# metno/gridpp

Hardware: AMD Instinct MI355X
Metric: grid cells/sec for optimal_interpolation, 4000x4000 grid, 10k obs (higher is better)
Workload: dtype f32 (rho, distances) + f64 (local solve)

## Files before the change

### gridpp_amd/csrc/oi_union.h

```cpp
#pragma once
#include "oi_common.h"

#pragma clang fp contract(off)

struct OiArgs {
    const float *gx, *gy, *gz, *gelev, *glaf, *bg, *bvar;
    float *out, *out_var;
    int C, ny, nx, tiles_x, ntiles, tiled2d;
    int wshift;
    ScanArgs s;
    const float4* ogeo;
    const float4* oaux;
    const float4* saux;
    int S, allow_extrap;
    int* err;
    unsigned long long* counters;
    const int* in_list;
    const int* in_count;
    int* out_list;
    int* out_count;
    int nrun;
    int tile0, tile_n;
    int* tail_count;
    const unsigned char* skip_flags;
    int level;
    const int* parent_count;
    int debug;
    int no_bulk_cert;
    int pair_solo;
    int* big_list;
    int* big_count;
    unsigned long long* big_keys;
    double* big_mat;
    int* huge_list;
    int* huge_count;
    unsigned long long* huge_keys;
    double* huge_mat;
    int huge_kcap, huge_ncap;
    unsigned* pair_sel;
    int* pair_n;
};

#define GPP_NSLOT 512
#define BIG_CAND 8192
#define BIG_N 512
#define BIG_NL 104
#define ERR_OVERFLOW 1
#define ERR_SINGULAR 2

__device__ __forceinline__ int nth_set_bit(unsigned long long mask, int m) {
    int pos = 0;
#pragma unroll
    for(int w = 32; w > 0; w >>= 1) {
        unsigned long long lowmask = (w == 32) ? 0xffffffffull : ((1ull << w) - 1ull);
        int c = __popcll((mask >> pos) & lowmask);
        if(m >= c) { m -= c; pos += w; }
    }
    return pos;
}

#ifdef GPP_UNION_STATS
#define UNION_STATS true
#else
#define UNION_STATS false
#endif
#ifdef GPP_UNION_PROFILE
#define UPROF(i) do { const unsigned long long t_ = __builtin_amdgcn_s_memtime(); if(lane == 0) L.prof[i] += (unsigned)(t_ - tprev); tprev = t_; } while(0)
#else
#define UPROF(i) do { } while(0)
#endif

template <int NC> struct UnionCfg;
template <> struct UnionCfg<32> {
    static constexpr int WCAP = 40;
    static constexpr int MAXU = 40;
    static constexpr int SOLVE = 1024;
#ifndef GPP_UNION_PERSIST
#define GPP_UNION_PERSIST 0
#endif
#ifndef GPP_UNION_WPB
#define GPP_UNION_WPB 2
#endif
    static constexpr int WPB = GPP_UNION_WPB;
    template <bool PLAIN> static constexpr bool persistent() { return PLAIN && GPP_UNION_PERSIST != 0; }
};
template <> struct UnionCfg<48> {
    static constexpr int WCAP = 56;
    static constexpr int MAXU = 56;
    static constexpr int SOLVE = 1792;
    static constexpr int WPB = 2;
    template <bool PLAIN> static constexpr bool persistent() { return false; }
};
template <> struct UnionCfg<64> {
    static constexpr int WCAP = 64;
    static constexpr int MAXU = 62;
    static constexpr int SOLVE = 2240;
    static constexpr int WPB = 2;
    template <bool PLAIN> static constexpr bool persistent() { return false; }
};
constexpr int U_MAXE = 12;
constexpr int U_MAXM = 6;

__device__ __forceinline__ unsigned union_xcd_order(const unsigned b, const unsigned nblocks) {
    const unsigned g = b & ~15u;
    if(g + 16u > nblocks) return b;
    const unsigned r = b & 15u;
    return g + ((r & 7u) << 1) + (r >> 3);
}

template <int NC>
struct UnionLds {
    static constexpr int U_WCAP = UnionCfg<NC>::WCAP, U_MAXU = UnionCfg<NC>::MAXU, U_SOLVE = UnionCfg<NC>::SOLVE;
    union {
        float rho[U_WCAP][64];
        struct {
            double solve[U_SOLVE];
            float erho[U_MAXE][64];
        } f;
    };
    int wpos[U_WCAP];
    int worig[U_WCAP];
#ifdef GPP_UNION_PROFILE
    unsigned prof[24];
#endif
    union {
        struct {
            float4 orec[U_MAXU];
            float olaf[U_MAXU];
        };
        double late[8][9];
    };
};

struct PairLds {
    int pos[2][UnionCfg<32>::WCAP];
    unsigned long long core[2];
    int state[2];
    int ok[2];
    float dmax, dmin;
};

#ifndef GPP_UNION_COLS
#define GPP_UNION_COLS 0
#endif
template <int NC, bool COLS>
__device__ __forceinline__ int union_solve_doubles(const int c, const int nE) {
    if constexpr(COLS) return c * (c + nE + 1) - c * (c - 1) / 2 + c + nE * nE + nE;
    else return c * (c + 1) / 2 + 2 * c + nE * (c | 1) + nE * nE + nE + 3;
}
__device__ __forceinline__ double rsqrt_nr(const double a) {
    double rs = __builtin_amdgcn_rsq(a);
    rs = rs * (1.5 - 0.5 * a * rs * rs);
    rs = rs * (1.5 - 0.5 * a * rs * rs);
    return rs;
}

template <bool PLAIN, bool LIST, int NC, bool PAIR = false, bool SP = false>
__device__ __forceinline__ void union_item(const OiArgs& a, int tile, int sub, const int shift, UnionLds<NC>& L, const int lane,
                                           const bool partner = false, const int pw = 0, const int lead = 0, UnionLds<NC>* const Lall = nullptr, PairLds* const PP = nullptr) {
    constexpr int U_WCAP = UnionCfg<NC>::WCAP, U_MAXU = UnionCfg<NC>::MAXU, U_SOLVE = UnionCfg<NC>::SOLVE;
    static_assert(!PAIR || (NC == 32 && !LIST), "the pair form exists for the first pass of the 32-column kernel only");
    static_assert(!SP || (PLAIN && NC == 32 && !PAIR), "the spatially varying form exists for the 32-column Barnes kernel only");
    tile = __builtin_amdgcn_readfirstlane(tile); sub = __builtin_amdgcn_readfirstlane(sub);
#ifdef GPP_UNION_PROFILE
    if(lane < 24) L.prof[lane] = 0u;
    unsigned long long tprev = __builtin_amdgcn_s_memtime();
#endif
    int cell = -1;
    if(a.tiled2d) {
        int ty = tile / a.tiles_x, tx = tile - ty * a.tiles_x;
        int y = ty * (64 >> a.wshift) + (lane >> a.wshift), x = (tx << a.wshift) + (lane & ((1 << a.wshift) - 1));
        if(y < a.ny && x < a.nx) cell = y * a.nx + x;
    }
    else {
        int c = tile * 64 + lane;
        if(c < a.C) cell = c;
    }
    if(LIST && (lane >> shift) != sub) cell = -1;
    float gx = 0, gy = 0, gz = 0, ge = NAN, gl = NAN, bg = NAN, bvar = 1.0f;
    if(cell >= 0) {
        gx = a.gx[cell]; gy = a.gy[cell]; gz = a.gz[cell]; ge = a.gelev[cell]; gl = a.glaf[cell];
        bg = a.bg[cell];
        if(a.bvar) bvar = a.bvar[cell];
    }
    const bool active = cell >= 0 && d_valid(bg);
    DevStructure st = a.s.st;
    const ScanArgs& sa = a.s;
    float sa_inv_s = sa.inv_s;
    if constexpr(SP) { if(cell >= 0) d_structure_at(st, st.cell_idx ? st.cell_idx[cell] : cell); }
    else if constexpr(!LIST) asm volatile("" : "+s"(st.h), "+s"(st.v), "+s"(st.w), "+s"(st.R), "+s"(sa_inv_s));

    UPROF(0);
    const float R = st.R;
    const int K = sa.K;
    const float h2 = st.h * st.h;
    const bool prune = PLAIN || st.kh == SK_BARNES;
    const float pa = sa.axis_a == 0 ? gx : (sa.axis_a == 1 ? gy : gz);
    const float pb = sa.axis_b == 1 ? gy : (sa.axis_b == 2 ? gz : gx);
    const float amin_t = wave_min(active ? pa : INFINITY), amax_t = wave_max(active ? pa : -INFINITY);
    const float bmin_t = wave_min(active ? pb : INFINITY), bmax_t = wave_max(active ? pb : -INFINITY);
    float emin_t = -INFINITY, emax_t = INFINITY, lmin_t = -INFINITY, lmax_t = INFINITY, kv2 = 0.0f, kw2 = 0.0f;
    if constexpr(PLAIN && !SP) {
        if(d_valid(st.v) && st.v != 0.0f && d_valid(st.h) && st.h != 0.0f) {
            emin_t = wave_min(active ? (d_valid(ge) ? ge : -INFINITY) : INFINITY); emax_t = wave_max(active ? (d_valid(ge) ? ge : INFINITY) : -INFINITY);
            kv2 = (st.h / st.v) * (st.h / st.v) * 0.9999f;
        }
        if(d_valid(st.w) && st.w != 0.0f && d_valid(st.h) && st.h != 0.0f) {
            lmin_t = wave_min(active ? (d_valid(gl) ? gl : -INFINITY) : INFINITY); lmax_t = wave_max(active ? (d_valid(gl) ? gl : INFINITY) : -INFINITY);
            kw2 = (st.h / st.w) * (st.h / st.w) * 0.9999f;
        }
    }
    int cnt = 0;
    unsigned long long mine = 0ull;
    unsigned long long alloc = 0ull;
    bool fb = false;
    bool cert = false;
    constexpr unsigned long long FULL = U_WCAP >= 64 ? ~0ull : ((1ull << (U_WCAP & 63)) - 1ull);
#pragma unroll
    for(int w = 0; w < U_WCAP; ++w) L.rho[w][lane] = INFINITY;
    auto live_mask = [&]() { return wave_or64(mine); };
    auto bulk_own = [&](const bool ok, const int s) {
        const unsigned okm = ok ? ~0u : 0u;
        const unsigned long long bit = 1ull << s;
        mine = ((unsigned long long)d_and_or_sc(okm, (unsigned)(bit >> 32), (unsigned)(mine >> 32)) << 32) | d_and_or_sc(okm, (unsigned)bit, (unsigned)mine);
        cnt -= (int)okm;
    };
    auto worst_slot = [&](float& r0, int& s0, bool& multi) {
        constexpr int NG = U_WCAP / 8;
        float gm[NG];
#pragma unroll
        for(int g = 0; g < NG; ++g) {
            float v[8];
#pragma unroll
            for(int j = 0; j < 8; ++j) v[j] = L.rho[8 * g + j][lane];
            gm[g] = fminf(fminf(fminf(v[0], v[1]), fminf(v[2], v[3])), fminf(fminf(v[4], v[5]), fminf(v[6], v[7])));
        }
        r0 = gm[0];
#pragma unroll
        for(int g = 1; g < NG; ++g) r0 = fminf(r0, gm[g]);
        int gs = 0, ng = 0;
#pragma unroll
        for(int g = 0; g < NG; ++g) { const bool eq = gm[g] == r0; gs = eq ? g : gs; ng += eq ? 1 : 0; }
        const float* const grp = &L.rho[0][lane] + gs * (8 * 64);
        float v[8];
#pragma unroll
        for(int j = 0; j < 8; ++j) v[j] = grp[j * 64];
        int sj = 0, nin = 0;
#pragma unroll
        for(int j = 0; j < 8; ++j) { const bool eq = v[j] == r0; sj = eq ? j : sj; nin += eq ? 1 : 0; }
        s0 = 8 * gs + sj;
        multi = ng > 1 || nin > 1;
    };
    if(wave_ballot(active) != 0ull) {
        const float sbin = 1.0f / sa_inv_s;
        int tby0 = (int)floorf((bmin_t - sa.bmin) * sa_inv_s), tby1 = (int)floorf((bmax_t - sa.bmin) * sa_inv_s);
        tby0 = __builtin_amdgcn_readfirstlane(min(max(tby0, 0), sa.nby - 1));
        tby1 = __builtin_amdgcn_readfirstlane(min(max(tby1, tby0), sa.nby - 1));
        int tbx0 = (int)floorf((amin_t - sa.amin) * sa_inv_s), tbx1 = (int)floorf((amax_t - sa.amin) * sa_inv_s);
        tbx0 = __builtin_amdgcn_readfirstlane(min(max(tbx0, 0), sa.nbx - 1));
        tbx1 = __builtin_amdgcn_readfirstlane(min(max(tbx1, tbx0), sa.nbx - 1));
        const float lox = gx - R, hix = gx + R, loy = gy - R, hiy = gy + R, loz = gz - R, hiz = gz + R;
        const float near_r = R - 4.76837158e-7f * (fabsf(gx) + fabsf(gy) + fabsf(gz) + R);
        float wr = 0.0f;
        int ws = 0;
        unsigned wo = 0u;
        const float thr2_R = R * R * 1.000001f + 1e-30f;
        float thr2 = active ? thr2_R : -1.0f;
        float bud2 = active ? INFINITY : -1.0f;

        const float ca = 0.5f * (amin_t + amax_t), cb = 0.5f * (bmin_t + bmax_t);
        const float rad = 0.5f * d_sqrt_raw((amax_t - amin_t) * (amax_t - amin_t) + (bmax_t - bmin_t) * (bmax_t - bmin_t)) * 1.001f + 1e-30f;
        auto proj_d2 = [&](const float4& rec) {
            const float ra = sa.axis_a == 0 ? rec.x : (sa.axis_a == 1 ? rec.y : rec.z);
            const float rb = sa.axis_b == 1 ? rec.y : (sa.axis_b == 2 ? rec.z : rec.x);
            return (ra - ca) * (ra - ca) + (rb - cb) * (rb - cb);
        };
        auto wave_lim2 = [&]() {
            const float t2 = __int_as_float(__builtin_amdgcn_readfirstlane(__float_as_int(wave_max(thr2))));
            if(t2 < 0.0f) return -1.0f;
            const float lim = (d_sqrt_raw(t2) + rad) * 1.0001f;
            return lim * lim;
        };

        const bool eprune = PLAIN && (kv2 != 0.0f || kw2 != 0.0f);
        auto wave_bud2 = [&]() { return eprune ? __int_as_float(__builtin_amdgcn_readfirstlane(__float_as_int(wave_max(bud2)))) : INFINITY; };
        auto keep = [&](const float pd, const float4& rec, const float2& met, const float lim2, const float B2) {
            bool k = pd <= lim2;
            if(eprune && B2 < INFINITY) {
                const float sd = fmaxf(d_sqrt_raw(pd) * 0.9999f - rad, 0.0f);
                const float dz = fmaxf(fmaxf(emin_t - rec.w, rec.w - emax_t), 0.0f), dl = fmaxf(fmaxf(lmin_t - met.x, met.x - lmax_t), 0.0f);
                k = k && (sd * sd + kv2 * dz * dz + kw2 * dl * dl <= B2);
            }
            return k;
        };

        const bool hv = d_valid(st.v) && st.v != 0.0f, hw = d_valid(st.w) && st.w != 0.0f, hh = d_valid(st.h) && st.h != 0.0f;
// ... 401 lines not shown
                if(UNION_STATS && lane == 0) atomicAdd(&a.counters[12], (unsigned long long)min(64, total - base));
                run_chunk(rec, met, pos, wave_ballot(keep(pd, rec, met, lim2, B2)));
            }
            const int nidx = 32 * (b + 1);
            if(nidx >= n0) {
                const int rn = 1 + ((nidx - n0) >> 1);
                const float t2n = __int_as_float(__builtin_amdgcn_readfirstlane(__float_as_int(wave_max(thr2))));
                const float gapn = (rn > 1) ? (float)(rn - 1) * sbin * 0.999f : 0.0f;
                if(t2n < 0.0f || gapn * gapn > t2n) break;
                if(tby0 - rn < 0 && tby1 + rn >= sa.nby) break;
            }
        }
    }

    UPROF(4);
    const unsigned long long upd = wave_ballot(cnt > 0);
    unsigned long long coreM = 0ull, extM = 0ull;
    int c = 0, nE = 0, u = 0;
    int m = 0;
    unsigned elist = 0u;
    if(!fb && upd != 0ull) {
        const bool up = cnt > 0;
        const unsigned long long unionM = wave_or64(up ? mine : 0ull);
        coreM = wave_and64(up ? mine : ~0ull);
        extM = unionM & ~coreM;
        if constexpr(UNION_STATS) {
            unsigned long long held = 0ull;
            for(int w = 0; w < U_WCAP; ++w) held |= (L.rho[w][lane] < INFINITY ? 1ull : 0ull) << w;
            if(wave_ballot(held != mine) != 0ull && lane == 0) atomicAdd(&a.counters[13], 1ull);
        }
    }
    int myslot = 0, mypos = 0;
    bool paired = false;
    if constexpr(PAIR) {
        if(partner) {
            PairLds& P = *PP;
            __builtin_amdgcn_fence(__ATOMIC_RELEASE, "wavefront");
            __builtin_amdgcn_wave_barrier();
            __builtin_amdgcn_fence(__ATOMIC_ACQUIRE, "wavefront");
            if(lane < U_WCAP) P.pos[pw][lane] = (((coreM | extM) >> lane) & 1ull) ? L.wpos[lane] : -1;
            if(lane == 0) { P.core[pw] = coreM; P.state[pw] = fb ? 2 : (upd == 0ull ? 1 : 0); }
            UPROF(11);
            __syncthreads();
            UPROF(12);
            if(P.state[0] == 0 && P.state[1] == 0) {
                const int pa = lane < U_WCAP ? P.pos[0][lane] : -1, pb = lane < U_WCAP ? P.pos[1][lane] : -1;
                int partB = -1, partA = -1;
#pragma unroll
                for(int t = 0; t < U_WCAP; ++t) {
                    const int qa = P.pos[0][t], qb = P.pos[1][t];
                    partB = (qb == pa) ? t : partB;
                    partA = (qa == pb) ? t : partA;
                }
                partB = pa >= 0 ? partB : -1;
                partA = pb >= 0 ? partA : -1;
                const unsigned long long coreA = P.core[0], coreB = P.core[1];
                const unsigned long long liveA = wave_ballot(pa >= 0);
                const unsigned long long pcore = wave_ballot(pa >= 0 && ((coreA >> lane) & 1ull) != 0ull && partB >= 0 && ((coreB >> (partB & 63)) & 1ull) != 0ull);
                const unsigned long long pextA = liveA & ~pcore;
                const unsigned long long bonly = wave_ballot(pb >= 0 && partA < 0);
                const int c2 = __popcll(pcore), nEa = __popcll(pextA), nE2 = nEa + __popcll(bonly), u2 = c2 + nE2;
                const bool fits = u2 <= U_MAXU && nE2 <= U_MAXE && union_solve_doubles<NC, (NC == 32 && GPP_UNION_COLS != 0) || SP>(c2, nE2) <= U_SOLVE;
                int sA = -1, sB = -1;
                {
                    const unsigned long long mk = lane < c2 ? pcore : (lane < c2 + nEa ? pextA : bonly);
                    const int idx = lane < c2 ? lane : (lane < c2 + nEa ? lane - c2 : lane - c2 - nEa);
                    const int sl = nth_set_bit(mk, idx);
                    if(lane < c2 + nEa) sA = sl; else if(lane < u2) sB = sl;
                }
                const int pbs = __shfl(partB, sA < 0 ? 0 : sA);
                if(sA >= 0) sB = pbs;
                const int posA = P.pos[0][sA < 0 ? 0 : sA], posB = P.pos[1][sB < 0 ? 0 : sB];
                const int slot2 = pw == 0 ? sA : sB, pos2 = sA >= 0 ? posA : posB;
                int m2 = 0;
                unsigned el2 = 0u;
                if(fits) {
#pragma unroll
                    for(int ai = 0; ai < U_MAXE; ++ai) {
                        if(ai < nE2) {
                            const int sl = __builtin_amdgcn_readlane(slot2, c2 + ai);
                            const bool sel = sl >= 0 && L.rho[sl < 0 ? 0 : sl][lane] < INFINITY;
                            if(sel) { el2 |= (unsigned)ai << (4 * (m2 & 7)); m2++; }
                        }
                    }
                }
                const bool ok = fits && wave_ballot(m2 > U_MAXM) == 0ull;
                if(lane == 0) P.ok[pw] = ok ? 1 : 0;
                UPROF(13);
                __syncthreads();
                UPROF(14);
                paired = P.ok[0] != 0 && P.ok[1] != 0;
                if(paired) { c = c2; nE = nE2; u = u2; m = m2; elist = el2; myslot = slot2; mypos = pos2; }
            }
        }
    }
    if(!paired && !fb && upd != 0ull) {
        c = __popcll(coreM); nE = __popcll(extM); u = c + nE;
        if(u > U_MAXU || nE > U_MAXE || union_solve_doubles<NC, (NC == 32 && GPP_UNION_COLS != 0) || SP>(c, nE) > U_SOLVE) {
            fb = true;
            if(UNION_STATS && lane == 0) atomicAdd(&a.counters[u > U_MAXU ? 5 : (nE > U_MAXE ? 6 : 7)], 1ull);
        }
        else {
            int ai = 0;
            for(unsigned long long mm = extM; mm; mm &= mm - 1ull, ++ai) {
                const int w = __builtin_ctzll(mm);
                if((mine >> w) & 1ull) { elist |= (unsigned)ai << (4 * (m & 7)); m++; }
            }
            if(wave_ballot(m > U_MAXM) != 0ull) { fb = true; if(UNION_STATS && lane == 0) atomicAdd(&a.counters[8], 1ull); }
        }
    }
    if(fb) {
        if(lane == 0) a.out_list[atomicAdd(a.out_count, 1)] = !LIST ? tile : (tile * 32 + (a.level == 1 ? 16 + sub : sub));
        return;
    }
    const bool solver = !PAIR || !paired || pw == lead;
    UnionLds<NC>& LS = (PAIR && paired) ? Lall[lead] : L;
    UPROF(5);
    float res_out = bg, res_var = bvar;
    if(upd != 0ull && !GPP_DBG(a, 1)) {
        if(!paired) {
            myslot = lane < c ? nth_set_bit(coreM, lane) : (lane < u ? nth_set_bit(extM, lane - c) : 0);
            mypos = L.wpos[myslot];
        }
        int oorig = 0;
        if constexpr(SP) oorig = L.worig[myslot];
        float4 o0 = make_float4(0, 0, 0, NAN), o1 = make_float4(NAN, 0, 0, 0);
        if(solver && lane < u) {
            o0 = sa.pgeo[mypos];
            o1 = a.saux[mypos];
        }
        const float dpf = (float)((double)o1.y - (double)o1.z);
        float gf[NC];
        {
            constexpr int NLATE = U_MAXU > NC ? U_MAXU - NC : 1;
            float gx8[NLATE];
            auto rho_of_row = [&](const int k) {
                const int sl = __builtin_amdgcn_readlane(myslot, k);
                if constexpr(PAIR) return sl >= 0 ? L.rho[sl][lane] : 0.0f;
                else return L.rho[sl][lane];
            };
#pragma unroll
            for(int k = 0; k < NC; ++k) gf[k] = (k < u) ? rho_of_row(k) : 0.0f;
#pragma unroll
            for(int k = NC; k < U_MAXU; ++k) gx8[k - NC] = (k < u) ? rho_of_row(k) : 0.0f;
            __builtin_amdgcn_wave_barrier();
#pragma unroll
            for(int k = 0; k < NC; ++k) if(k >= c && k < u) L.f.erho[k - c][lane] = gf[k];
#pragma unroll
            for(int k = NC; k < U_MAXU; ++k) if(k < u) L.f.erho[k - c][lane] = gx8[k - NC];
        }
        if(solver && lane >= c && lane < u) L.worig[lane - c] = __float_as_int(dpf);
        UPROF(6);
        constexpr bool COLS = NC == 32 && GPP_UNION_COLS != 0;
        const int FAC = c * (u + 1) - c * (c - 1) / 2;
        const int oL = 0, oI = (COLS || SP) ? FAC : c * (c + 1) / 2, oZ = oI + c, oB = oZ + c, bs = c | 1, oS = (COLS || SP) ? oI + c : oB + nE * bs, oD = oS + nE * nE;
        double* const sv = LS.f.solve;
        bool bad = false;
        float maxInc = -INFINITY, minInc = INFINITY;
        double inc = 0.0, a00 = 0.0;
        const int mmax = __builtin_amdgcn_readfirstlane((int)wave_max((float)m));
        if constexpr(SP) {
            const DevStructure& su = a.s.st;
            float* const colbuf = reinterpret_cast<float*>(L.f.solve);
            double* const rsc = L.f.solve + 800;
            float* const rR = reinterpret_cast<float*>(L.f.solve + 920);
            if(lane < u) {
                const int fi = su.obs_idx[oorig];
                const float h_i = su.fh[fi], v_i = su.fv[fi], w_i = su.fw[fi];
                rsc[lane] = (d_valid(h_i) && h_i != 0.0f) ? 1.0 / (double)h_i : 0.0;
                rsc[40 + lane] = (d_valid(v_i) && v_i != 0.0f) ? 1.0 / (double)v_i : 0.0;
                rsc[80 + lane] = (d_valid(w_i) && w_i != 0.0f) ? 1.0 / (double)w_i : 0.0;
                rR[lane] = su.fR[fi];
                L.orec[lane] = o0; L.olaf[lane] = o1.x;
            }
            const bool anyv = wave_ballot(lane < u && rsc[40 + (lane < u ? lane : 0)] != 0.0) != 0ull, anyw = wave_ballot(lane < u && rsc[80 + (lane < u ? lane : 0)] != 0.0) != 0ull;
            __builtin_amdgcn_fence(__ATOMIC_RELEASE, "wavefront");
            __builtin_amdgcn_wave_barrier();
            __builtin_amdgcn_fence(__ATOMIC_ACQUIRE, "wavefront");
            const int nent = u * u;
            for(int e0 = 0; e0 < nent; e0 += 64) {
                const int e = min(e0 + lane, nent - 1);
                const int i = (int)(((float)e + 0.5f) / (float)u), pcol = e - i * u;
                const float4 ri = L.orec[i], rp = L.orec[pcol];
                const float hd = d_chord(ri.x, ri.y, ri.z, rp.x, rp.y, rp.z);
                float cv = d_barnes_rho_flat(hd, rsc[i]);
                if(anyv) { const float f = d_barnes_rho_flat((d_valid(ri.w) && d_valid(rp.w)) ? ri.w - rp.w : 0.0f, rsc[40 + i]); cv = (d_valid(ri.w) && d_valid(rp.w)) ? cv * f : cv; }
                if(anyw) { const float li = L.olaf[i], lp = L.olaf[pcol]; const float f = d_barnes_rho_flat((d_valid(li) && d_valid(lp)) ? li - lp : 0.0f, rsc[80 + i]); cv = (d_valid(li) && d_valid(lp)) ? cv * f : cv; }
                cv = hd > rR[i] ? 0.0f : cv;
                if(e0 + lane < nent) colbuf[pcol * U_MAXU + i] = cv;
            }
            __builtin_amdgcn_fence(__ATOMIC_RELEASE, "wavefront");
            __builtin_amdgcn_wave_barrier();
            __builtin_amdgcn_fence(__ATOMIC_ACQUIRE, "wavefront");
            UPROF(7);
            double row[NC];
#pragma unroll
            for(int p = 0; p < NC; ++p) {
                double v = 0.0;
                if(p < u && lane < u) { v = (double)colbuf[p * U_MAXU + lane]; if(lane == p) v += (double)o1.w; }
                row[p] = v;
            }
            float lt[8];
#pragma unroll
            for(int b = 0; b < 8; ++b) lt[b] = (32 + b < u && lane < u) ? colbuf[(32 + b) * U_MAXU + lane] : 0.0f;
            const double dcol = lane < u ? (double)o1.y - (double)o1.z : 0.0;
            __builtin_amdgcn_fence(__ATOMIC_RELEASE, "wavefront");
            __builtin_amdgcn_wave_barrier();
            __builtin_amdgcn_fence(__ATOMIC_ACQUIRE, "wavefront");
            auto rcp_nr = [](const double x) { double r = __builtin_amdgcn_rcp(x); r = r * (2.0 - x * r); r = r * (2.0 - x * r); return r; };
            {
                int co = 0;
#pragma unroll
                for(int j = 0; j < NC; ++j) {
                    if(j < c) {
                        const double piv = readlane_d(row[j], j);
                        if(!(fabs(piv) > 1e-290)) bad = true;
                        const double rp = rcp_nr(piv);
                        if(lane == j) {
                            sv[oI + j] = rp;
#pragma unroll
                            for(int p = j; p < NC; ++p) if(p < u) sv[co + p - j] = row[p];
                        }
                        const double mlt = lane > j ? row[j] * rp : 0.0;
                        if(lane > j) row[j] = mlt;
                        __builtin_amdgcn_fence(__ATOMIC_RELEASE, "wavefront");
                        __builtin_amdgcn_wave_barrier();
                        __builtin_amdgcn_fence(__ATOMIC_ACQUIRE, "wavefront");
                        const double* const q = sv + co - j;
#pragma unroll
                        for(int p = j + 1; p < NC; ++p) row[p] = __builtin_fma(-mlt, q[p], row[p]);
                        co += u + 1 - j;
                    }
                }
            }
            UPROF(8);
            const int ea = lane - c;
            const int myco = lane * (u + 1) - lane * (lane - 1) / 2;
            auto subst = [&](double t) {
#pragma unroll
                for(int j = 0; j < NC; ++j) {
                    if(j < c) { const double tj = readlane_d(t, j); t = lane > j ? __builtin_fma(-row[j], tj, t) : t; }
                }
                return t;
            };
#pragma unroll
            for(int b = 0; b < 8; ++b) {
                const int p = 32 + b;
                if(p < u) {
                    const double t = subst((double)lt[b] + (lane == p ? (double)o1.w : 0.0));
                    if(lane < c) sv[myco + p - lane] = t;
                    else if(lane < u) sv[oS + ea * nE + (p - c)] = t;
                }
            }
            {
                const double t = subst(dcol);
                if(lane < c) sv[myco + u - lane] = t;
                else if(lane < u) sv[oD + ea] = t;
            }
#pragma unroll
            for(int p = 0; p < NC; ++p) {
                if(p >= c && p < u) { if(lane >= c && lane < u) sv[oS + ea * nE + (p - c)] = row[p]; }
            }
            if(!a.allow_extrap) {
                maxInc = wave_max(lane < c ? dpf : -INFINITY);
                minInc = wave_min(lane < c ? dpf : INFINITY);
            }
            __builtin_amdgcn_fence(__ATOMIC_RELEASE, "wavefront");
            __builtin_amdgcn_wave_barrier();
            __builtin_amdgcn_fence(__ATOMIC_ACQUIRE, "wavefront");
            UPROF(9);
            double z[NC];
#pragma unroll
            for(int k = 0; k < NC; ++k) z[k] = (double)gf[k];
            double qx[U_MAXM];
            const double* xp[U_MAXM];
#pragma unroll
            for(int i = 0; i < U_MAXM; ++i) {
                const int ai = (elist >> (4 * i)) & 15;
                qx[i] = (i < mmax) ? (double)L.f.erho[ai][lane] : 0.0;
                xp[i] = sv + c + ai;
            }
            {
                int co = 0;
#pragma unroll
                for(int j = 0; j < NC; ++j) {
                    if(j < c) {
                        const double* const ur = sv + co - j;
                        const double zj = z[j] * sv[oI + j];
                        inc = __builtin_fma(zj, ur[u], inc);
#pragma unroll
                        for(int k = j + 1; k < NC; ++k) z[k] = __builtin_fma(-ur[k], zj, z[k]);
#pragma unroll
                        for(int i = 0; i < U_MAXM; ++i) if(i < mmax) { qx[i] = __builtin_fma(-*xp[i], zj, qx[i]); xp[i] += u - j; }
                        co += u + 1 - j;
                    }
                }
            }
            if(mmax > 0) {
                double lu[U_MAXM][U_MAXM], iu[U_MAXM], tq[U_MAXM], yd[U_MAXM];
#pragma unroll
                for(int i = 0; i < U_MAXM; ++i) {
                    if(i < mmax) {
                        const int ai = (elist >> (4 * i)) & 15;
                        const bool valid = i < m;
#pragma unroll
                        for(int jj = 0; jj < U_MAXM; ++jj) {
                            if(jj < mmax) {
                                const int aj = (elist >> (4 * jj)) & 15;
                                double sij = sv[oS + ai * nE + aj];
#pragma unroll
                                for(int k = 0; k < (i < jj ? i : jj); ++k) sij = __builtin_fma(-lu[i][k], lu[k][jj], sij);
                                lu[i][jj] = jj < i ? sij * iu[jj] : sij;
                            }
                        }
                        if(valid && !(fabs(lu[i][i]) > 1e-290)) bad = true;
                        iu[i] = rcp_nr(valid ? lu[i][i] : 1.0);
                        double y = sv[oD + ai], t = qx[i];
#pragma unroll
                        for(int k = 0; k < i; ++k) { y = __builtin_fma(-lu[i][k], yd[k], y); t = __builtin_fma(-lu[k][i], tq[k], t); }
                        yd[i] = y;
                        tq[i] = t * iu[i];
                        if(valid) {
                            inc = __builtin_fma(tq[i], yd[i], inc);
                            if(!a.allow_extrap) {
                                const float de = __int_as_float(LS.worig[ai]);
                                maxInc = fmaxf(maxInc, de); minInc = fminf(minInc, de);
                            }
                        }
                    }
                }
            }
        }
        else {
        if(solver) {
        if(lane < u) { L.orec[lane] = o0; L.olaf[lane] = o1.x; }
        float* colbuf = reinterpret_cast<float*>(L.f.solve);
        const int ntri = u * (u + 1) / 2;
#ifndef GPP_UNION_PB
#define GPP_UNION_PB 1
#endif
        constexpr int PB = PLAIN ? GPP_UNION_PB : 1;
        const bool hh = d_valid(st.h) && st.h != 0.0f, hv = d_valid(st.v) && st.v != 0.0f, hw = d_valid(st.w) && st.w != 0.0f;
        const double rh = hh ? 1.0 / (double)st.h : 0.0, rv_ = hv ? 1.0 / (double)st.v : 0.0, rw_ = hw ? 1.0 / (double)st.w : 0.0;
        for(int e0 = 0; e0 < ntri; e0 += 64 * PB) {
            int ti[PB], tp[PB];
            float4 ri[PB], rp[PB];
            float li[PB], lp[PB];
#pragma unroll
            for(int q = 0; q < PB; ++q) {
                const int e = min(e0 + 64 * q + lane, ntri - 1);
                int i = (int)((d_sqrt_raw(8.0f * (float)e + 1.0f) - 1.0f) * 0.5f);
                if(i * (i + 1) / 2 > e) i--;
                if((i + 1) * (i + 2) / 2 <= e) i++;
                ti[q] = i; tp[q] = e - i * (i + 1) / 2;
                ri[q] = L.orec[ti[q]]; rp[q] = L.orec[tp[q]];
                li[q] = L.olaf[ti[q]]; lp[q] = L.olaf[tp[q]];
            }
            float cv[PB];
            if constexpr(PLAIN) {
                float hd[PB];
#pragma unroll
                for(int q = 0; q < PB; ++q) { hd[q] = d_chord(ri[q].x, ri[q].y, ri[q].z, rp[q].x, rp[q].y, rp[q].z); cv[q] = 1.0f; }
                if(hh) {
#pragma unroll
                    for(int q = 0; q < PB; ++q) cv[q] = d_barnes_rho_flat(hd[q], rh);
                }
                if(hv) {
#pragma unroll
                    for(int q = 0; q < PB; ++q) { const float f = d_barnes_rho_flat(ri[q].w - rp[q].w, rv_); cv[q] = (d_valid(ri[q].w) && d_valid(rp[q].w)) ? cv[q] * f : cv[q]; }
                }
                if(hw) {
#pragma unroll
                    for(int q = 0; q < PB; ++q) { const float f = d_barnes_rho_flat(li[q] - lp[q], rw_); cv[q] = (d_valid(li[q]) && d_valid(lp[q])) ? cv[q] * f : cv[q]; }
                }
#pragma unroll
                for(int q = 0; q < PB; ++q) cv[q] = hd[q] > st.R ? 0.0f : cv[q];
            }
            else {
#pragma unroll
                for(int q = 0; q < PB; ++q) cv[q] = d_corr_t<PLAIN>(st, ri[q].x, ri[q].y, ri[q].z, ri[q].w, li[q], rp[q].x, rp[q].y, rp[q].z, rp[q].w, lp[q], false);
            }
#pragma unroll
            for(int q = 0; q < PB; ++q) if(e0 + 64 * q + lane < ntri) colbuf[tp[q] * U_MAXU + ti[q]] = cv[q];
        }
        double* const colL = L.f.solve + (U_SOLVE - 64);
        if(lane < u) colL[lane] = (double)o1.y - (double)o1.z;
        __builtin_amdgcn_fence(__ATOMIC_RELEASE, "wavefront");
        __builtin_amdgcn_wave_barrier();
        __builtin_amdgcn_fence(__ATOMIC_ACQUIRE, "wavefront");
        UPROF(7);
        double row[NC];
#pragma unroll
        for(int p = 0; p < NC; ++p) {
            double v = 0.0;
            if(p < u) {
                if(lane < u && lane >= p) {
                    v = (double)colbuf[p * U_MAXU + lane];
                    if(lane == p) v += (double)o1.w;
                }
                if(lane == 63) v = colL[p];
            }
            row[p] = v;
        }
        const int lidx = lane == 63 ? 8 : lane - NC;
#pragma unroll
        for(int b = 0; b < (U_MAXU > NC ? 8 : 0); ++b) {
            const int p = NC + b;
            if(p < u) {
                double v = 0.0;
                if(lane < u && lane >= p) {
                    v = (double)colbuf[p * U_MAXU + lane];
                    if(lane == p) v += (double)o1.w;
                }
                if(lane == 63) v = colL[p];
                if((lane >= p && lane < u) || lane == 63) L.late[b][lidx] = v;
            }
        }
        __builtin_amdgcn_wave_barrier();
        if constexpr(COLS) {
        int co = 0;
#pragma unroll
        for(int j = 0; j < NC; j += 2) {
            if(j < c) {
                const bool two = j + 1 < c;
                const double pa = readlane_d(row[j], j), pb = readlane_d(row[j], j + 1), pc = readlane_d(row[j + 1], j + 1);
                const double det = two ? __builtin_fma(pa, pc, -(pb * pb)) : 1.0;
                if(!(pa > 0.0) || !(det > 0.0)) bad = true;
                const double r1 = rsqrt_nr(pa), rd = rsqrt_nr(det);
                const double l21 = pb * r1, i22 = two ? rd * (pa * r1) : 0.0;
                const double c1 = row[j] * r1;
                const double t2 = __builtin_fma(-c1, l21, row[j + 1]);
                const double c2 = t2 * i22;
                row[j] = c1;
                row[j + 1] = two ? c2 : t2;
                const int co1 = co + (u + 1 - j);
                if(lane == 0) { sv[oI + j] = r1; if(two) sv[oI + j + 1] = i22; }
                {
                    const int r = lane == 63 ? u : lane;
                    if((lane >= j && lane < u) || lane == 63) sv[co + r - j] = c1;
                    if(two && ((lane > j && lane < u) || lane == 63)) sv[co1 + r - (j + 1)] = c2;
                }
                const double* const q1 = sv + co - j;
                const double* const q2 = two ? sv + co1 - (j + 1) : q1;
#pragma unroll
                for(int p = j + 2; p < NC; ++p) {
                    row[p] = __builtin_fma(-c1, q1[p], row[p]);
                    row[p] = __builtin_fma(-c2, q2[p], row[p]);
                }
                co = co1 + (u - j);
            }
        }
        UPROF(8);
        const int ea = lane - c;
        {
            const bool erow = lane >= c && lane < u;
            const int bse = (erow ? oS + ea * nE : oD) - c;
#pragma unroll
            for(int p = 0; p < NC; ++p) {
                if(p >= c && p < u) { if((erow && p <= lane) || lane == 63) sv[bse + p] = row[p]; }
            }
        }
        if(u > 32 && !GPP_DBG(a, 16)) {
            __builtin_amdgcn_fence(__ATOMIC_RELEASE, "wavefront");
            __builtin_amdgcn_wave_barrier();
            __builtin_amdgcn_fence(__ATOMIC_ACQUIRE, "wavefront");
#pragma unroll
            for(int b = 0; b < 8; ++b) {
                const int p = 32 + b;
                if(p < u) {
                    const bool mine = (lane >= p && lane < u) || lane == 63;
                    double acc = mine ? L.late[b][lidx] : 0.0;
                    int ck = p;
#pragma unroll
                    for(int k = 0; k < 32; ++k) {
                        if(k < c) acc = __builtin_fma(-row[k], sv[ck], acc);
                        ck += u - k;
                    }
                    if(lane >= p && lane < u) sv[oS + ea * nE + (p - c)] = acc;
                    else if(lane == 63) sv[oD + (p - c)] = acc;
                }
            }
        }
        }
        else {
#pragma unroll
        for(int j = 0; j < NC; ++j) {
            if(j < c) {
                const double ajj = readlane_d(row[j], j);
                if(!(ajj > 0.0)) bad = true;
                const double rs = rsqrt_nr(ajj);
                if(lane == 0) sv[oI + j] = rs;
                const double cj = row[j] * rs;
                row[j] = cj;
                colL[lane] = cj;
                {
                    static_assert(NC % 2 == 0 && (U_SOLVE - 64) % 2 == 0, "colL and its pairs are 16-byte aligned");
                    const int pe = (j + 2) & ~1;
                    if(pe != j + 1) row[j + 1] = __builtin_fma(-cj, colL[j + 1], row[j + 1]);
                    typedef double d2v __attribute__((ext_vector_type(2)));
                    const d2v* const colL2 = reinterpret_cast<const d2v*>(colL);
#pragma unroll
                    for(int p = pe; p < NC; p += 2) {
                        const d2v v = colL2[p >> 1];
                        row[p] = __builtin_fma(-cj, v.x, row[p]);
                        row[p + 1] = __builtin_fma(-cj, v.y, row[p + 1]);
                    }
                }
            }
        }
        UPROF(8);
        int ce = c, ue = u;
        asm("" : "+s"(ce), "+s"(ue));
        const int ea = lane - c;
        {
            int maxp = -1, baseLo = 0, baseHi = 0;
            if(lane < c) { maxp = lane; baseLo = oL + lane * (lane + 1) / 2; baseHi = baseLo; }
            else if(lane < u) { maxp = u - 1; baseLo = oB + ea * bs; baseHi = oS + ea * nE - c; }
            else if(lane == 63) { maxp = u - 1; baseLo = oZ; baseHi = oD - c; }
#pragma unroll
            for(int p = 0; p < NC; ++p) {
                const int bse = (p < ce) ? baseLo : baseHi;
                if(p <= maxp) sv[bse + p] = row[p];
            }
        }
        if(U_MAXU > NC && ue > NC && !GPP_DBG(a, 16)) {
            __builtin_amdgcn_fence(__ATOMIC_RELEASE, "wavefront");
            __builtin_amdgcn_wave_barrier();
            __builtin_amdgcn_fence(__ATOMIC_ACQUIRE, "wavefront");
#pragma unroll
            for(int b = 0; b < 8; ++b) {
                const int p = NC + b;
                if(p < ue) {
                    const bool mine = (lane >= p && lane < u) || lane == 63;
                    double acc = mine ? L.late[b][lidx] : 0.0;
                    const double* const bp = sv + oB + (p - c) * bs;
#pragma unroll
                    for(int k = 0; k < NC; k += 4) {
                        if(k + 3 < ce) {
                            const double b0 = bp[k], b1 = bp[k + 1], b2 = bp[k + 2], b3 = bp[k + 3];
                            acc = __builtin_fma(-row[k], b0, acc);
                            acc = __builtin_fma(-row[k + 1], b1, acc);
                            acc = __builtin_fma(-row[k + 2], b2, acc);
                            acc = __builtin_fma(-row[k + 3], b3, acc);
                        }
                        else if(k < ce) {
                            acc = __builtin_fma(-row[k], bp[k], acc);
                            if(k + 1 < ce) acc = __builtin_fma(-row[k + 1], bp[k + 1], acc);
                            if(k + 2 < ce) acc = __builtin_fma(-row[k + 2], bp[k + 2], acc);
                        }
                    }
                    if(lane >= p && lane < u) sv[oS + ea * nE + (p - c)] = acc;
                    else if(lane == 63) sv[oD + (p - c)] = acc;
                }
            }
        }
        if(lane >= c && lane < u && (c & 1) == 0) sv[oB + ea * bs + c] = 0.0;
        if(lane < 3) sv[oD + nE + lane] = 0.0;
        }
        if(!a.allow_extrap) {
            maxInc = wave_max(lane < c ? dpf : -INFINITY);
            minInc = wave_min(lane < c ? dpf : INFINITY);
        }
        if constexpr(PAIR) {
            if(paired) {
                if(lane == 0) { PP->dmax = maxInc; PP->dmin = minInc; }
                if(bad && lane == 0) atomicOr(a.err, ERR_SINGULAR);
                bad = false;
            }
        }
        __builtin_amdgcn_fence(__ATOMIC_RELEASE, "wavefront");
        __builtin_amdgcn_wave_barrier();
        __builtin_amdgcn_fence(__ATOMIC_ACQUIRE, "wavefront");
        }
        if constexpr(PAIR) {
            if(paired) {
                UPROF(9);
                __syncthreads();
                UPROF(15);
                if(!solver) { maxInc = PP->dmax; minInc = PP->dmin; }
            }
        }

        UPROF(9);
        if constexpr(COLS) {
        double z[NC];
#pragma unroll
        for(int k = 0; k < NC; ++k) z[k] = (double)gf[k];
        double qx[U_MAXM];
        const double* xp[U_MAXM];
#pragma unroll
        for(int i = 0; i < U_MAXM; ++i) {
            const int ai = (elist >> (4 * i)) & 15;
            qx[i] = (i < mmax) ? (double)L.f.erho[ai][lane] : 0.0;
            xp[i] = sv + c + ai;
        }
        {
            int co = 0;
#pragma unroll
            for(int k = 0; k < NC; ++k) {
                if(k < c && !GPP_DBG(a, 32)) {
                    const double* const col = sv + co - k;
                    const double zk = z[k] * sv[oI + k];
                    inc = __builtin_fma(zk, col[u], inc);
                    a00 = __builtin_fma(zk, zk, a00);
#pragma unroll
                    for(int i = k + 1; i < NC; ++i) z[i] = __builtin_fma(-col[i], zk, z[i]);
#pragma unroll
                    for(int i = 0; i < U_MAXM; ++i) if(i < mmax) { qx[i] = __builtin_fma(-*xp[i], zk, qx[i]); xp[i] += u - k; }
                    co += u + 1 - k;
                }
            }
        }
        if(mmax > 0 && !GPP_DBG(a, 64)) {
            double ll[U_MAXM * (U_MAXM + 1) / 2], qv[U_MAXM], tv[U_MAXM], il[U_MAXM];
#pragma unroll
            for(int i = 0; i < U_MAXM; ++i) {
                if(i < mmax) {
                    const int ai = (elist >> (4 * i)) & 15;
                    const bool valid = i < m;
                    double gq = qx[i];
                    double dq = sv[oD + ai];
                    double sii = sv[oS + ai * nE + ai];
#pragma unroll
                    for(int jj = 0; jj < i; ++jj) {
                        const int aj = (elist >> (4 * jj)) & 15;
                        double sij = sv[oS + ai * nE + aj];
#pragma unroll
                        for(int k = 0; k < jj; ++k) sij = __builtin_fma(-ll[i * (i + 1) / 2 + k], ll[jj * (jj + 1) / 2 + k], sij);
                        const double lij = sij * il[jj];
                        ll[i * (i + 1) / 2 + jj] = lij;
                        sii = __builtin_fma(-lij, lij, sii);
                        gq = __builtin_fma(-lij, qv[jj], gq);
                        dq = __builtin_fma(-lij, tv[jj], dq);
                    }
                    if(valid && !(sii > 0.0)) bad = true;
                    const double rs = rsqrt_nr(valid ? sii : 1.0);
                    il[i] = rs;
                    qv[i] = gq * rs;
                    tv[i] = dq * rs;
                    if(valid) {
                        inc = __builtin_fma(qv[i], tv[i], inc);
                        a00 = __builtin_fma(qv[i], qv[i], a00);
                        if(!a.allow_extrap) {
                            const float de = __int_as_float(LS.worig[ai]);
                            maxInc = fmaxf(maxInc, de); minInc = fminf(minInc, de);
                        }
                    }
                }
            }
        }
        }
        else {
        int cf = c;
        asm("" : "+s"(cf));
        double z[NC];
#pragma unroll
        for(int k = 0; k < NC; ++k) {
            double zk = 0.0;
            if(k < cf && !GPP_DBG(a, 32)) {
                const double gk = (double)gf[k];
                double acc0 = 0.0, acc1 = 0.0;
                const double* lrow = sv + oL + k * (k + 1) / 2;
#pragma unroll
                for(int j = 0; j < k; ++j) {
                    if(j & 1) acc1 = __builtin_fma(lrow[j], z[j], acc1);
                    else acc0 = __builtin_fma(lrow[j], z[j], acc0);
                }
                zk = (gk - (acc0 + acc1)) * sv[oI + k];
                inc = __builtin_fma(zk, sv[oZ + k], inc);
            }
            z[k] = zk;
        }
        const bool want_var = a.out_var != nullptr;
        if(want_var) {
#pragma unroll
            for(int k = 0; k < NC; ++k) a00 = __builtin_fma(z[k], z[k], a00);
        }
        if(mmax > 0 && !GPP_DBG(a, 64)) {
            double ll[U_MAXM * (U_MAXM + 1) / 2], qv[U_MAXM], tv[U_MAXM], il[U_MAXM];
#pragma unroll
            for(int i = 0; i < U_MAXM; ++i) {
                if(i < mmax) {
                    const int ai = (elist >> (4 * i)) & 15;
                    const bool valid = i < m;
                    const double gi = (double)L.f.erho[ai][lane];
                    const double* brow = sv + oB + ai * bs;
                    double acc0 = 0.0, acc1 = 0.0;
#pragma unroll
                    for(int j0 = 0; j0 < NC; j0 += 4) {
                        if(j0 < cf) {
                            acc0 = __builtin_fma(brow[j0], z[j0], acc0);
                            acc1 = __builtin_fma(brow[j0 + 1], z[j0 + 1], acc1);
                            acc0 = __builtin_fma(brow[j0 + 2], z[j0 + 2], acc0);
                            acc1 = __builtin_fma(brow[j0 + 3], z[j0 + 3], acc1);
                        }
                    }
                    double gq = gi - (acc0 + acc1);
                    double dq = sv[oD + ai];
                    double sii = sv[oS + ai * nE + ai];
#pragma unroll
                    for(int jj = 0; jj < i; ++jj) {
                        const int aj = (elist >> (4 * jj)) & 15;
                        double sij = sv[oS + ai * nE + aj];
#pragma unroll
                        for(int k = 0; k < jj; ++k) sij = __builtin_fma(-ll[i * (i + 1) / 2 + k], ll[jj * (jj + 1) / 2 + k], sij);
// ... 158 lines not shown
```

Baseline: 4.397 billion.

## Split Cholesky row registers across idle upper lanes of the wave

For the 32-column non-pair path, each row of the local Cholesky factorization is split between two lanes. The lower lane keeps the first 18 columns and an otherwise idle upper lane (lanes 40..62) keeps the upper columns. The goal is to cut the per-lane double register array from 32 to 18 entries, which lowers VGPR pressure and may raise occupancy. In exchange it adds cross-lane shuffles for the late-column accumulations, extra LDS traffic for multipliers and more complex indexing, all of which carry correctness risk.

```diff
diff --git a/gridpp_amd/csrc/oi_union.h b/gridpp_amd/csrc/oi_union.h
--- a/gridpp_amd/csrc/oi_union.h
+++ b/gridpp_amd/csrc/oi_union.h
@@ -142,6 +142,9 @@
 
 #ifndef GPP_UNION_COLS
 #define GPP_UNION_COLS 0
+#endif
+#ifndef GPP_UNION_SPLIT
+#define GPP_UNION_SPLIT 1
 #endif
 template <int NC, bool COLS>
 __device__ __forceinline__ int union_solve_doubles(const int c, const int nE) {
@@ -849,6 +852,7 @@
         if(solver && lane >= c && lane < u) L.worig[lane - c] = __float_as_int(dpf);
         UPROF(6);
         constexpr bool COLS = NC == 32 && GPP_UNION_COLS != 0;
+        constexpr bool SPLIT = NC == 32 && !PAIR && !SP && !COLS && GPP_UNION_SPLIT != 0;
         const int FAC = c * (u + 1) - c * (c - 1) / 2;
         const int oL = 0, oI = (COLS || SP) ? FAC : c * (c + 1) / 2, oZ = oI + c, oB = oZ + c, bs = c | 1, oS = (COLS || SP) ? oI + c : oB + nE * bs, oD = oS + nE * nE;
         double* const sv = LS.f.solve;
@@ -1086,7 +1090,30 @@
         __builtin_amdgcn_wave_barrier();
         __builtin_amdgcn_fence(__ATOMIC_ACQUIRE, "wavefront");
         UPROF(7);
-        double row[NC];
+        constexpr int HS = SPLIT ? 18 : NC, HO = NC - HS, HL = U_MAXU - HS;
+        static_assert(!SPLIT || (2 * U_MAXU - HS + 2 == 64 && HO % 2 == 0 && 2 * HS >= NC + 4), "rows and their upper halves fill the wave; pairs of multipliers stay 16-byte aligned");
+        const bool up = SPLIT && lane >= U_MAXU && lane < 63;
+        const int orow = up ? (lane == 62 ? 63 : lane - HL) : lane;
+        const int cofs = up ? HO : 0;
+        double row[HS];
+        if constexpr(SPLIT) {
+            const float rdiag = __shfl(o1.w, orow);
+            const int rk = orow < u ? orow - cofs : -1;
+            const int dk = lane >= 62 ? u - cofs : 0;
+            const float* const cb = colbuf + cofs * U_MAXU + (orow < u ? orow : 0);
+            const double* const cd = colL + cofs;
+#pragma unroll
+            for(int k = 0; k < HS; ++k) {
+                double v = 0.0;
+                if(k <= rk) {
+                    v = (double)cb[k * U_MAXU];
+                    if(k == rk) v += (double)rdiag;
+                }
+                if(k < dk) v = cd[k];
+                row[k] = v;
+            }
+        }
+        else {
 #pragma unroll
         for(int p = 0; p < NC; ++p) {
             double v = 0.0;
@@ -1098,6 +1125,7 @@
                 if(lane == 63) v = colL[p];
             }
             row[p] = v;
+        }
         }
         const int lidx = lane == 63 ? 8 : lane - NC;
 #pragma unroll
@@ -1180,6 +1208,64 @@
         }
         }
         else {
+        if constexpr(SPLIT) {
+        typedef double d2v __attribute__((ext_vector_type(2)));
+        static_assert((U_SOLVE - 64) % 2 == 0, "colL and its pairs are 16-byte aligned");
+        const double* const cm = colL + cofs;
+        double* const cw = colL + lane;
+        double* const cr = colL + orow;
+#pragma unroll
+        for(int j = 0; j < NC; ++j) {
+            if(j < c) {
+                if(j < HS) {
+                    const double ajj = readlane_d(row[j], j);
+                    if(!(ajj > 0.0)) bad = true;
+                    const double rs = rsqrt_nr(ajj);
+                    if(lane == 0) sv[oI + j] = rs;
+                    *cw = row[j] * rs;
+                    const double cj = *cr;
+                    if(!up) row[j] = cj;
+                    constexpr int K4 = 4;
+                    const int k0 = j + 1 < K4 ? j + 1 : K4;
+                    double mv[HS];
+                    const int pe = (k0 + 1) & ~1;
+                    if(pe != k0) mv[k0] = cm[k0];
+#pragma unroll
+                    for(int k = pe; k < HS; k += 2) {
+                        const d2v v = reinterpret_cast<const d2v*>(cm)[k >> 1];
+                        mv[k] = v.x; mv[k + 1] = v.y;
+                    }
+#pragma unroll
+                    for(int k = j + 1; k < HS; ++k) row[k] = __builtin_fma(-cj, mv[k], row[k]);
+                    if(up) {
+#pragma unroll
+                        for(int k = K4; k <= j; ++k) row[k] = __builtin_fma(-cj, mv[k], row[k]);
+                    }
+                }
+                else {
+                    const int s = j - HO;
+                    const double ajj = readlane_d(row[s], j + HL);
+                    if(!(ajj > 0.0)) bad = true;
+                    const double rs = rsqrt_nr(ajj);
+                    if(lane == 0) sv[oI + j] = rs;
+                    if(up) {
+                        const double cj = row[s] * rs;
+                        row[s] = cj;
+                        *cr = cj;
+                        const int pe = (s + 2) & ~1;
+                        if(pe != s + 1) row[s + 1] = __builtin_fma(-cj, cm[s + 1], row[s + 1]);
+#pragma unroll
+                        for(int k = pe; k < HS; k += 2) {
+                            const d2v v = reinterpret_cast<const d2v*>(cm)[k >> 1];
+                            row[k] = __builtin_fma(-cj, v.x, row[k]);
+                            row[k + 1] = __builtin_fma(-cj, v.y, row[k + 1]);
+                        }
+                    }
+                }
+            }
+        }
+        }
+        else {
 #pragma unroll
         for(int j = 0; j < NC; ++j) {
             if(j < c) {
@@ -1205,11 +1291,32 @@
                 }
             }
         }
+        }
         UPROF(8);
         int ce = c, ue = u;
         asm("" : "+s"(ce), "+s"(ue));
         const int ea = lane - c;
-        {
+        const int eo = orow - c;
+        if constexpr(SPLIT) {
+            int maxp = -1, baseLo = 0, baseHi = 0;
+            if(orow < c) { maxp = orow; baseLo = oL + orow * (orow + 1) / 2; baseHi = baseLo; }
+            else if(orow < u) { maxp = u - 1; baseLo = oB + eo * bs; baseHi = oS + eo * nE - c; }
+            else if(orow == 63) { maxp = u - 1; baseLo = oZ; baseHi = oD - c; }
+            const int maxk = maxp - cofs, ck = ce - cofs;
+            baseLo += cofs; baseHi += cofs;
+#pragma unroll
+            for(int k = 0; k < HS; ++k) {
+                const int bse = (k < ck) ? baseLo : baseHi;
+                if(k <= maxk && (k >= 2 * HS - NC || !up)) sv[bse + k] = row[k];
+            }
+            if(ce < HS && ue > HS) {
+                if(lane >= c && lane < HS) {
+#pragma nounroll
+                    for(int p = HS; p < min(ue, NC); ++p) sv[oS + ea * nE + (p - c)] = 0.0;
+                }
+            }
+        }
+        else {
             int maxp = -1, baseLo = 0, baseHi = 0;
             if(lane < c) { maxp = lane; baseLo = oL + lane * (lane + 1) / 2; baseHi = baseLo; }
             else if(lane < u) { maxp = u - 1; baseLo = oB + ea * bs; baseHi = oS + ea * nE - c; }
@@ -1231,6 +1338,37 @@
                     const bool mine = (lane >= p && lane < u) || lane == 63;
                     double acc = mine ? L.late[b][lidx] : 0.0;
                     const double* const bp = sv + oB + (p - c) * bs;
+                    if constexpr(SPLIT) {
+                        auto part = [&](const int k, const int sl) {
+                            if(k + 3 < ce) {
+                                const double b0 = bp[k], b1 = bp[k + 1], b2 = bp[k + 2], b3 = bp[k + 3];
+                                acc = __builtin_fma(-row[sl], b0, acc);
+                                acc = __builtin_fma(-row[sl + 1], b1, acc);
+                                acc = __builtin_fma(-row[sl + 2], b2, acc);
+                                acc = __builtin_fma(-row[sl + 3], b3, acc);
+                            }
+                            else if(k < ce) {
+                                acc = __builtin_fma(-row[sl], bp[k], acc);
+                                if(k + 1 < ce) acc = __builtin_fma(-row[sl + 1], bp[k + 1], acc);
+                                if(k + 2 < ce) acc = __builtin_fma(-row[sl + 2], bp[k + 2], acc);
+                            }
+                        };
+#pragma unroll
+                        for(int k = 0; k + 3 < HS; k += 4) part(k, k);
+#pragma unroll
+                        for(int k = HS & ~3; k < HS; ++k) if(k < ce) acc = __builtin_fma(-row[k], bp[k], acc);
+                        static_assert(NC + 1 - U_MAXE > HS, "the chain of a late column ends in the upper half");
+                        acc = __hiloint2double(__shfl(__double2hiint(acc), orow), __shfl(__double2loint(acc), orow));
+#pragma unroll
+                        for(int k = HS; k < ((HS + 3) & ~3); ++k) if(k < ce) acc = __builtin_fma(-row[k - HO], bp[k], acc);
+#pragma unroll
+                        for(int k = (HS + 3) & ~3; k < NC; k += 4) part(k, k - HO);
+                        if(up) {
+                            if(orow >= p && orow < u) sv[oS + eo * nE + (p - c)] = acc;
+                            else if(orow == 63) sv[oD + (p - c)] = acc;
+                        }
+                    }
+                    else {
 #pragma unroll
                     for(int k = 0; k < NC; k += 4) {
                         if(k + 3 < ce) {
@@ -1248,6 +1386,7 @@
                     }
                     if(lane >= p && lane < u) sv[oS + ea * nE + (p - c)] = acc;
                     else if(lane == 63) sv[oD + (p - c)] = acc;
+                    }
                 }
             }
         }
```

Measured after the change: 4.660 billion (median of 6 runs). +6.0%, better.
